# RaduAlexandru/permuto_sdf

Measured on AMD Instinct MI355X. Metric: ray-samples/sec (encode+MLP+composite), higher is better.
Workload: dtype f32 (MLP products on 2 fp16 operand pieces per fp32 value, fp32 accumulation; the 3-piece / 24-bit figure is value_fp32_equivalent_24bit)

## Files before the change

### include/psdf.h

```cpp
#ifndef PSDF_H
#define PSDF_H
#include <stdint.h>
#ifdef __cplusplus
extern "C" {
#endif

int64_t psdf_encode_convention(int which);
int psdf_encode_set_conventions(uint32_t hash_multiplier, int rank_tie_raises_later);

int psdf_encode_forward(int pos_dim, int nr_feat, int64_t N, int nr_levels, int capacity, const float* positions,
    const float* lattice, const float* scale_factor, const float* shifts, const float* window, int concat_points,
    float points_scaling, float* sliced, void* stream);

int psdf_encode_forward_mark(int pos_dim, int nr_feat, int64_t N, int nr_levels, int capacity, const float* positions,
    const float* lattice, const float* scale_factor, const float* shifts, const float* window, int concat_points,
    float points_scaling, float* sliced, unsigned char* touched_blocks, int block_rows_log2, void* stream);

int psdf_encode_backward(int pos_dim, int nr_feat, int64_t N, int nr_levels, int capacity, const float* positions,
    const float* lattice, const float* scale_factor, const float* shifts, const float* window, int concat_points,
    float points_scaling, const float* grad_sliced, float* grad_lattice, float* grad_positions, void* stream);

int64_t psdf_encode_backward_workspace_bytes(int pos_dim, int nr_feat, int64_t N, int nr_levels, int capacity);
int psdf_encode_backward_ws(int pos_dim, int nr_feat, int64_t N, int nr_levels, int capacity, const float* positions,
    const float* lattice, const float* scale_factor, const float* shifts, const float* window, int concat_points,
    float points_scaling, const float* grad_sliced, float* grad_lattice, float* grad_positions, void* workspace,
    int64_t workspace_bytes, void* stream);
int psdf_encode_backward_level_shares(int* counts, int max_levels);


int psdf_encode_double_backward(int pos_dim, int nr_feat, int64_t N, int nr_levels, int capacity, const float*
    positions, const float* lattice, const float* scale_factor, const float* shifts, const float* window, int
    concat_points, float points_scaling, const float* dd_positions, const float* grad_sliced, float* grad_lattice,
    float* grad_grad_sliced, void* stream);
int psdf_encode_double_backward_ws(int pos_dim, int nr_feat, int64_t N, int nr_levels, int capacity, const float* positions,
                                   const float* lattice, const float* scale_factor, const float* shifts, const float* window,
                                   int concat_points, float points_scaling, const float* dd_positions, const float* grad_sliced,
                                   float* grad_lattice, float* grad_grad_sliced, const float* grad_sliced_direct,
                                   void* workspace, int64_t workspace_bytes, void* stream);

int psdf_mlp_pack_f16(int n_layers, const int* dims, const float* const* weights, const float* const* biases, float* packed,
    void* stream);
int psdf_mlp_forward_f16(int n_layers, const int* dims, int64_t N, const float* X, const float* packed, float* Y, void* stream);

int psdf_neus_composite_forward(int nr_rays, const int* start_end, int equal, int fixed, int max_nr_samples, const float* sdf,
    const float* dirs, const float* gradients, const float* dt, const float* rgb, const float* inv_s, float cos_anneal_ratio,
    float* pred, float* bg, float* weights, void* stream);
int psdf_neus_composite_backward(int nr_rays, const int* start_end, int equal, int fixed, int max_nr_samples, int max_per_ray,
    const float* grad_pred, const float* grad_bg, const float* sdf, const float* dirs, const float* gradients, const float* dt,
    const float* rgb, const float* inv_s, float cos_anneal_ratio, int reference_compat, float* grad_sdf, float* grad_gradients,
    float* grad_rgb, float* grad_inv_s, void* stream);

int psdf_nerf_composite_forward(int nr_rays, const int* start_end, int equal, int fixed, int max_nr_samples, const float* raw_density,
                                const float* dt, const float* rgb, const float* fg_pred, const float* fg_bg, float* pred_bg,
                                float* pred, void* stream);
int psdf_nerf_composite_backward(int nr_rays, const int* start_end, int equal, int fixed, int max_nr_samples, int max_per_ray,
                                 const float* grad_pred, const float* fg_bg, const float* raw_density, const float* dt,
                                 const float* rgb, int reference_compat, float* grad_raw_density, float* grad_rgb,
                                 float* grad_fg_bg, void* stream);

int psdf_last_path(int family);
enum {
  PSDF_MLP_OP_FORWARD = 0,
  PSDF_MLP_OP_FORWARD_F16 = 1,
  PSDF_MLP_OP_FORWARD_WIDE_F16 = 2,
  PSDF_MLP_OP_BACKWARD = 3,
  PSDF_MLP_OP_BACKWARD_DATA = 4,
  PSDF_MLP_OP_BACKWARD_DATA_MASKED = 5,
  PSDF_MLP_OP_DOUBLE_BACKWARD = 6,
  PSDF_MLP_OP_DOUBLE_BACKWARD_PLUS = 7
};
int psdf_mlp_supported(int op, int n_layers, const int* dims);

int psdf_mlp_backward_split(int n_layers, const int* dims, int64_t N, const float* X, const float* const* weights,
    const float* const* biases, const float* dY, float* dX, float* const* dW, float* const* db, void* stream);

int psdf_mlp_backward_split_f16(int n_layers, const int* dims, int64_t N, const float* X, const float* const* weights,
    const float* const* biases, const float* dY, float* dX, float* const* dW, float* const* db, void* stream);
int psdf_mlp_backward_split_f16_form(void);
unsigned psdf_mlp_f16_range_events(void);

int psdf_mlp_forward_wide_f16(int n_layers, const int* dims, int64_t N, const float* X, const float* const* weights,
    const float* const* biases, float* Y, void* stream);
int psdf_mlp_backward_wide_form(void);
int psdf_mlp_backward_wide(int n_layers, const int* dims, int64_t N, const float* X, const float* const* weights,
    const float* const* biases, const float* dY, float* dX, float* const* dW, float* const* db, void* stream);

int psdf_lipshitz_normalize_forward(int out, int in, const float* W, const float* c, float* Wn, void* stream);
int psdf_lipshitz_normalize_backward(int out, int in, const float* W, const float* c, const float* grad_Wn, float* grad_W,
    float* grad_c, void* stream);
int psdf_lipshitz_normalize_forward_multi(int n_layers, const int* out, const int* in, const float* const* W, const float* const* c,
                                          float* const* Wn, void* stream);
int psdf_lipshitz_normalize_backward_multi(int n_layers, const int* out, const int* in, const float* const* W, const float* const* c,
                                           const float* const* grad_Wn, float* const* grad_W, float* const* grad_c, void* stream);

int psdf_neus_alpha_forward(int64_t N, const float* sdf, const float* dirs, const float* gradients, const float* dt,
    const float* inv_s, float cos_anneal_ratio, float* alpha, float* one_minus_alpha, void* stream);
int psdf_neus_alpha_backward(int64_t N, const float* grad_alpha, const float* sdf, const float* dirs, const float*
    gradients, const float* dt, const float* inv_s, float cos_anneal_ratio, float* grad_sdf, float* grad_gradients,
    float* grad_inv_s, void* stream);
int psdf_l1_loss(int64_t R, int C, const float* pred, const float* gt, const unsigned char* mask, float scale,
    float* loss, float* grad_pred, void* stream);
int psdf_eikonal_loss(int64_t N, const float* gradients, float scale, float* loss, float* grad_gradients, void* stream);
int psdf_normalize3(int64_t N, const float* x, const float* grad_y, float* out, void* stream);
int psdf_sigmoid_rows(int64_t N, int C, const float* x_fm, float* y, void* stream);
int psdf_sigmoid_rows_backward(int64_t N, int C, const float* grad_y, const float* y, float* grad_x_fm, void* stream);
int psdf_curvature_shift(int64_t N, const float* points, const float* gradients, const float* rand_directions, float
    epsilon, const float* grad_shifted, float* out, void* stream);
int psdf_curvature_loss(int64_t N, const float* gradients, const float* gradients_shifted, float scale, float* loss,
    float* grad_gradients, float* grad_gradients_shifted, void* stream);
int psdf_offsurface_loss(int64_t N, const float* sdf, float sharpness, float scale, float* loss, float* grad_sdf, void*
    stream);
int psdf_nerf_alpha_forward(int64_t N, const float* raw_density, const float* dt, float* alpha, float* one_minus_alpha,
    void* stream);
int psdf_nerf_alpha_backward(int64_t N, const float* raw_density, const float* dt, const float* grad_alpha, const float*
    grad_one_minus_alpha, float* grad_raw_density, void* stream);

int64_t psdf_mlp_packed_size(int n_layers, const int* dims);

int psdf_mlp_pack(int n_layers, const int* dims, const float* const* weights, const float* const* biases, float*
    packed, void* stream);

int psdf_mlp_forward(int n_layers, const int* dims, int64_t N, const float* X, const float* packed, float* Y, void*
    stream);

int psdf_encode_forward_masked(int pos_dim, int nr_feat, int64_t N, int nr_levels, int capacity, const float* positions,
    const float* lattice, const float* scale_factor, const float* shifts, const float* window, int concat_points, float
    points_scaling, const uint8_t* skip, float* sliced, void* stream);
int psdf_mlp_forward_masked(int n_layers, const int* dims, int64_t N, const float* X, const float* packed, const uint8_t*
    skip, float* Y, void* stream);
int psdf_mlp_backward_data_masked(int n_layers, const int* dims, int64_t N, const float* X, const float* const* weights,
    const float* const* biases, const float* dY, const uint8_t* skip, float* dX, void* stream);
int psdf_encode_backward_positions_masked(int pos_dim, int nr_feat, int64_t N, int nr_levels, int capacity, const float*
    positions, const float* lattice, const float* scale_factor, const float* shifts, const float* window, int
    concat_points, float points_scaling, const float* grad_sliced, const uint8_t* skip, float* grad_positions, void*
    stream);

int psdf_mlp_backward(int n_layers, const int* dims, int64_t N, const float* X, const float* const* weights, const
    float* const* biases, const float* dY, float* dX, float* const* dW, float* const* db, void* stream);

int psdf_mlp_double_backward(int n_layers, const int* dims, int64_t N, const float* X, const float* const* weights,
    const float* const* biases, const float* dY, const float* V, float* dX2, float* const* dW, float* const* db,
    void* stream);
int psdf_mlp_double_backward_plus(int n_layers, const int* dims, int64_t N, const float* X, const float* const* weights,
    const float* const* biases, const float* dY, const float* V, const float* dY2, float* dX2, float* const* dW,
    float* const* db, void* stream);

int psdf_encode_mlp_forward(int64_t N, int nr_levels, int capacity, const float* positions, const float* lattice,
    const float* scale_factor, const float* shifts, const float* window, int concat_points, float points_scaling,
    int n_layers, const int* dims, const float* packed, const uint8_t* skip, float* feat, float* Y, void* stream);

int psdf_adamw_step(int64_t n, float* param, const float* grad, float* exp_avg, float* exp_avg_sq, float lr, float
    beta1, float beta2, float eps, float weight_decay, int step, float grad_scale, void* stream);

int psdf_adamw_step_multi(int n_tensors, const int64_t* sizes, float* const* params, const float* const* grads, float*
    const* exp_avgs, float* const* exp_avg_sqs, float lr, float beta1, float beta2, float eps, float weight_decay, int
    step, float grad_scale, void* stream);

int psdf_adamw_step_blocks(int64_t n_blocks, int block_elems, float* param, float* grad, float* exp_avg, float*
    exp_avg_sq, unsigned char* touched, unsigned char* active, float lr, float beta1, float beta2, float eps, int step,
    float grad_scale, int zero_grad, void* stream);
int psdf_adamw_step_blocks_multi(int n_tensors, const int64_t* n_blocks, const int* block_elems, float* const* params,
    float* const* grads, float* const* exp_avgs, float* const* exp_avg_sqs, unsigned char* const* touched,
    unsigned char* const* active, const float* lr, const float* beta1, const float* beta2, const float* eps, const int* step,
    float grad_scale, int zero_grad, void* stream);


int psdf_grid_points(int count, int nr_voxels_per_dim, float extent, const float* grid_translation, const int*
    voxel_indices, uint64_t rng_state, uint64_t rng_inc, int randomize, float* out_points, void* stream);

int psdf_grid_update_with_density(int count, const int* voxel_indices, const float* density, float decay, float
    thresh, float* grid_values, uint8_t* grid_occupancy, void* stream);

int psdf_grid_update_with_sdf(int count, const int* voxel_indices, const float* sdf, int nr_voxels_per_dim, float
    extent, const float* grid_translation, float inv_s, const float* inv_s_tensor, int full_update, float thresh,
    float* grid_values, uint8_t* grid_occupancy, void* stream);

int psdf_grid_check_occupancy(int count, int nr_voxels_per_dim, float extent, const float* grid_translation, const
    uint8_t* grid_occupancy, const float* points, uint8_t* out, void* stream);

int psdf_march_form(void);
int psdf_march_samples(int use_grid, int nr_rays, int nr_voxels_per_dim, float extent, const float* grid_translation,
    const uint8_t* grid_occupancy, const float* ray_origins, const float* ray_dirs, const float* ray_t_entry, const
    float* ray_t_exit, float min_dist_between_samples, int max_nr_samples_per_ray, int max_nr_samples, uint64_t
    rng_state, uint64_t rng_inc, int jitter, float* samples_pos, float* samples_dirs, float* samples_z, float*
    samples_dt, float* ray_fixed_dt, int* ray_start_end_idx, int* cur_nr_samples, int* scratch, const uint32_t*
    coarse_mask, void* stream);

int psdf_first_hit_samples(int nr_rays, int nr_voxels_per_dim, float extent, const float* grid_translation, const
    uint8_t* grid_occupancy, const float* ray_origins, const float* ray_dirs, const float* ray_t_entry, const float*
    ray_t_exit, int max_nr_samples, float* samples_pos, float* samples_dirs, float* samples_z, float* samples_dt,
    float* ray_fixed_dt, int* ray_start_end_idx, int* cur_nr_samples, int* scratch, const uint32_t* coarse_mask,
    void* stream);

int psdf_advance_to_next_occupied_voxel(int count, int nr_voxels_per_dim, float extent, const float* grid_translation,
    const uint8_t* grid_occupancy, const float* samples_dirs, float* samples_pos, uint8_t* is_within_bounds, const
    uint32_t* coarse_mask, void* stream);

int psdf_occupancy_coarse_words(int nr_voxels_per_dim);
int psdf_occupancy_coarse_mask(int nr_voxels_per_dim, const uint8_t* grid_occupancy, uint32_t* coarse_mask, void*
    stream);

int psdf_samples_bg(int nr_rays, int nr_samples_per_ray, const float* ray_origins, const float* ray_dirs, const float*
    ray_t_exit, float sphere_radius, const float* sphere_center, uint64_t rng_state, uint64_t rng_inc, int randomize,
    int contract_3d_samples, float* samples_3d, float* samples_4d, float* samples_dirs, float* samples_z, float*
    samples_dt, float* ray_fixed_dt, int* ray_start_end_idx, void* stream);

int psdf_sphere_ray_intersection(int nr_rays, float radius, const float* center, const float* ray_origins, const
    float* ray_dirs, float* points_entry, float* t_entry, float* points_exit, float* t_exit, uint8_t* does_intersect,
    void* stream);

int psdf_sphere_rand_points_inside(int count, float radius, const float* phi, const float* costheta, const float* u,
    float* points, void* stream);

int psdf_compact_offsets(int nr_rays, const int* ray_start_end_idx, int* scratch, int* total, void* stream);

int psdf_compact_copy(int nr_rays, const int* ray_start_end_idx, const int* offsets, const float* pos, const float*
    pos4, const float* dirs, const float* z, const float* dt, const float* sdf, const float* fixed_dt, float* o_pos,
    float* o_pos4, float* o_dirs, float* o_z, float* o_dt, float* o_sdf, float* o_fixed_dt, int* o_start_end, void*
    stream);

int psdf_per_sample_ray_idx(int nr_rays, int nr_samples, const int* ray_start_end_idx, int* out, void* stream);

int psdf_spherical_harmonics(int count, int degree, const float* dirs, float* out, void* stream);

int psdf_random_rays_from_reel(int nr_rays, int nr_images, int height, int width, const float* rgb_reel, const float*
    mask_reel, const float* K_reel, const float* tf_world_cam_reel, const int* pixel_indices, const int* img_indices,
    int has_mask, float* ray_origins, float* ray_dirs, float* gt_rgb, float* gt_mask, void* stream);

int psdf_first_hit_dense(int nr_rays, int nr_voxels_per_dim, float extent, const float* grid_translation, const
    uint8_t* grid_occupancy, const float* ray_origins, const float* ray_dirs, const float* ray_t_entry, const float*
    ray_t_exit, float* pos, uint8_t* converged, const uint32_t* coarse_mask, void* stream);
int psdf_sphere_trace_step(int count, int nr_voxels_per_dim, float extent, const float* grid_translation, const
    uint8_t* grid_occupancy, const float* dirs, const float* sdf, float sdf_multiplier, float sdf_converged_thresh,
    float* pts, uint8_t* converged, const uint32_t* coarse_mask, void* stream);
int psdf_sphere_trace_step_compacted(int count, int nr_voxels_per_dim, float extent, const float* grid_translation, const
    uint8_t* grid_occupancy, const float* dirs, const float* sdf, float sdf_multiplier, float sdf_converged_thresh,
    float* pts, uint8_t* converged, uint8_t* work_flags, int* work_list, int* work_count, const uint32_t* coarse_mask,
    void* stream);

int psdf_exclusive_scan_i32(int n, const int* in, int* out, int* total, void* stream);

int psdf_cumprod_alpha2transmittance(int nr_rays, const int* start_end, int equal, int fixed, int max_nr_samples,
    const float* alpha, float* transmittance, float* bg_transmittance, void* stream);

int psdf_cumprod_alpha2transmittance_backward(int nr_rays, const int* start_end, int equal, int fixed, int
    max_nr_samples, const float* grad_bg, const float* alpha, const float* bg, const float* cumsumLV, float*
    grad_alpha, void* stream);

int psdf_integrate_with_weights(int nr_rays, const int* start_end, int equal, int fixed, int max_nr_samples, const
    float* rgb, const float* weights, float* pred, void* stream);

int psdf_integrate_with_weights_backward(int nr_rays, const int* start_end, int equal, int fixed, int max_nr_samples,
    const float* grad_pred, const float* rgb, const float* weights, float* grad_rgb, float* grad_weights, int
    reference_compat, void* stream);

int psdf_sum_over_each_ray(int nr_rays, const int* start_end, int equal, int fixed, int max_nr_samples, int channels,
    const float* values, float* sum_per_ray, float* sum_per_sample, void* stream);

int psdf_sum_over_each_ray_backward(int nr_rays, const int* start_end, int equal, int fixed, int max_nr_samples, int
    channels, const float* grad_per_ray, const float* grad_per_sample, float* grad_values, void* stream);

int psdf_cumsum_over_each_ray(int nr_rays, const int* start_end, int equal, int fixed, int max_nr_samples, const
    float* values, int inverse, int exclusive, float* out, void* stream);

int psdf_sdf2alpha(int nr_rays, const int* start_end, int equal, int fixed, int max_nr_samples, const float*
    ray_fixed_dt, const float* samples_dt, const float* sdf, float inv_s, int dynamic_inv_s, float inv_s_multiplier,
    float* alpha, void* stream);
int psdf_sdf_importance_cdf(int nr_rays, const int* start_end, int equal, int fixed, int max_nr_samples, const float* ray_fixed_dt,
                            const float* samples_dt, const float* sdf, float inv_s, int dynamic_inv_s, float inv_s_multiplier,
                            float* cdf, void* stream);

int psdf_compute_dt(int nr_rays, const int* start_end, int equal, int fixed, int max_nr_samples, const float*
    samples_z, const float* ray_t_exit, int use_ray_t_exit, float* dt, void* stream);

int psdf_volume_render_nerf(int nr_rays, const int* start_end, int equal, int fixed, int max_nr_samples, const float*
    rgb, const float* density, const float* samples_z, const float* samples_dt, float* pred_rgb, float* pred_depth,
    float* bg_transmittance, float* weight_per_sample, void* stream);

int psdf_volume_render_nerf_backward(int nr_rays, const int* start_end, int equal, int fixed, int max_nr_samples,
    const float* grad_pred_rgb, const float* grad_bg_transmittance, const float* pred_rgb, const float*
    bg_transmittance, const float* rgb, const float* density, const float* samples_dt, float* grad_rgb, float*
    grad_density, void* stream);

int psdf_importance_sample(int nr_rays, const int* start_end, int equal, int fixed, int max_nr_samples, const float*
    ray_origins, const float* ray_dirs, const float* ray_fixed_dt, const float* samples_z, const float* cdf, int
    nr_importance_samples, uint64_t rng_state, uint64_t rng_inc, int jitter, float* out_pos, float* out_dirs, float*
    out_z, void* stream);

int psdf_combine_uniform_samples_with_imp(int nr_rays, const int* uni_start_end, int uni_equal, int uni_fixed, int
    uni_max_nr_samples, const float* ray_origins, const float* ray_dirs, const float* ray_t_exit, const float*
    uni_fixed_dt, const float* uni_z, const float* uni_sdf, int has_sdf, int nr_imp, const float* imp_z, const float*
    imp_sdf, int out_max_nr_samples, float* out_pos, float* out_dirs, float* out_z, float* out_dt, float* out_sdf,
    float* out_fixed_dt, int* out_start_end, int* out_cur_nr_samples, int* scratch, void* stream);

int psdf_mesh_classify(const float* vol, const uint8_t* valid, float level, int X, int Y, int Z, int xbase, int nplanes, int p0,
    int p1, int c0, int c1, uint8_t* mask, int32_t* vcount, int32_t* tcount, void* stream);
int psdf_mesh_emit_vertices(const float* vol, float level, int X, int Y, int Z, int xbase, int nplanes, int p0, int p1, const
    uint8_t* mask, const int32_t* vincl, int64_t v_off, float* verts, int64_t* edges, float* normals, void* stream);
int psdf_mesh_emit_faces(const float* vol, const uint8_t* valid, float level, int X, int Y, int Z, int xbase, int nplanes, int c0,
    int c1, const uint8_t* mask, const int32_t* vincl, const int32_t* tincl, int32_t* faces, void* stream);
int psdf_mesh_grid_points(int nx, int Y, int Z, int x0, int64_t first, int64_t count, const float* xs, const float* ys, const
    float* zs, float* points, void* stream);
int psdf_mesh_sparse_mask(int64_t count, int nr_voxels_per_dim, float extent, const float* grid_translation, const uint8_t*
    grid_occupancy, const float* points, float h, uint8_t* valid, uint8_t* skip, void* stream);

int psdf_mesh_eval_tile_capacity(void);
int psdf_mesh_eval_grid_plan(const double* lo, const double* hi, int64_t n_points, double min_edge, int64_t cell_budget, float*
    origin_edge, int* dims, int64_t* cells, int64_t* query_blocks);
int psdf_mesh_sample_count(const float* V, int64_t nV, const int32_t* F, int64_t nF, double density, int32_t* counts, int32_t*
    overflow, void* stream);
int psdf_mesh_sample_emit(const float* V, int64_t nV, const int32_t* F, int64_t nF, double density, const int64_t* incl, float*
    samples, void* stream);
int psdf_mesh_eval_cell_keys(const float* points, int64_t n, const float* origin_edge, const int* dims, int block_log2, int32_t*
    keys, void* stream);
int psdf_mesh_eval_cell_ranges(const int32_t* sorted_keys, int64_t n, int64_t cells, int32_t* start, void* stream);
int psdf_mesh_thin_sweep(const float* points, const int32_t* rank, const int32_t* keys, int64_t n, const int32_t* cell_start,
    const float* origin_edge, const int* dims, float radius, uint8_t* state, int32_t* undecided, void* stream);
int psdf_mesh_nn_cooperative(const float* queries, int64_t nq, const int32_t* query_block_start, const float* refs, int64_t nr,
    const int32_t* cell_start, const float* origin_edge, const int* dims, float max_dist, float* dist, int32_t* idx, uint8_t*
    open, int32_t* nr_open, void* stream);
int psdf_mesh_nn_ring(const float* queries, int64_t nq, const float* refs, int64_t nr, const int32_t* cell_start, const float*
    origin_edge, const int* dims, float max_dist, float* dist, int32_t* idx, const uint8_t* open, void* stream);

#ifdef __cplusplus
}
#endif
#endif
```

### permuto_sdf_amd/csrc/mlp.hip

```cpp
#include "psdf_common.h"

#include "mlp_device.h"
#include "mlp_dispatch.h"

namespace {

struct PackArgs {
  MlpPlan plan;
  const float* W[MAXL];
  const float* b[MAXL];
};

__global__ void mlp_pack_kernel(PackArgs a, float* __restrict__ packed) {
  const int e = blockIdx.x * blockDim.x + threadIdx.x;
  const MlpPlan& p = a.plan;
  if (e >= p.total) return;
  int l = 0;
#pragma unroll
  for (int i = 1; i < MAXL; i++)
    if (i < p.n_layers && e >= p.w_off[i]) l = i;
  const int out_d = p.dims[l + 1], in_d = p.dims[l];
  const bool last = (l == p.n_layers - 1);
  float v = 0.f;
  if (e >= p.b_off[l]) {
    const int row = e - p.b_off[l];
    if (row < out_d) v = a.b[l][row];
  } else {
    const int q = e - p.w_off[l];
    int row, col;
    if (l == 0) {
      const int lane = q % WS, s = (q / WS) % p.in_steps0, to = (q / WS) / p.in_steps0;
      row = (lane < 64) ? 32 * to + (lane & 31) : (1 << 20);
      col = 2 * s + (lane >> 5);
    } else if (last && p.final_dot) {
      const int h = q & 1, r = (q >> 1) & 15, ti = (q >> 5) % p.tiles[l], o = (q >> 5) / p.tiles[l];
      row = o;
      col = 32 * ti + row_of(r, h);
    } else {
      const int j = q & 3, lane = (q >> 2) & 63, rq = (q >> 8) & 3, pr = q >> 10;
      const int r = 4 * rq + j, ti = pr % p.tiles[l], to = pr / p.tiles[l];
      row = 32 * to + (lane & 31);
      col = 32 * ti + row_of(r, lane >> 5);
    }
    if (row < out_d && col < in_d) v = a.W[l][(int64_t)row * in_d + col];
  }
  packed[e] = v;
}

__global__ void mlp_pack_split_kernel(PackArgs a, SplitPlan sp, float* __restrict__ packed, int f16) {
  const int w = blockIdx.x * blockDim.x + threadIdx.x;
  const MlpPlan& p = a.plan;
  if (w >= sp.total_rec * 4) return;
  uint32_t* dst = reinterpret_cast<uint32_t*>(packed + sp.base);
  const int nl = p.n_layers;
  const int rec = w >> 2;
  if (rec >= sp.tail_rec) {
    const int f = w - sp.tail_rec * 4;
    float v = 0.f;
    for (int l = 0; l < nl; l++) {
      const bool dot = (l == nl - 1) && p.final_dot;
      const int nb = dot ? 4 : p.tiles[l + 1] * 32;
      if (f >= sp.b_off[l] && f < sp.b_off[l] + nb) {
        const int row = f - sp.b_off[l];
        if (row < p.dims[l + 1]) v = a.b[l][row];
      }
      if (dot && f >= sp.wf_off && f < sp.wf_off + p.dims[nl] * p.tiles[l] * 32) {
        const int q = f - sp.wf_off;
        const int h = q & 1, r = (q >> 1) & 15, ti = (q >> 5) % p.tiles[l], o = (q >> 5) / p.tiles[l];
        const int col = 32 * ti + row_of(r, h);
        if (col < p.dims[l]) v = a.W[l][(int64_t)o * p.dims[l] + col];
      }
    }
    dst[w] = __float_as_uint(v);
    return;
  }
  int l = 0;
  for (int i = 1; i < nl; i++) {
    const bool dot = (i == nl - 1) && p.final_dot;
    if (!dot && rec >= sp.w_rec[i]) l = i;
  }
  const int local = rec - sp.w_rec[l];
  const int lane = local & 63, piece = (local >> 6) % 3, s = (local / 192) % sp.ns[l], to = (local / 192) / sp.ns[l];
  const int row = 32 * to + (lane & 31), hh = lane >> 5;
  uint32_t out = 0;
  for (int e = 0; e < 2; e++) {
    const int j = 2 * (w & 3) + e;
    const int col = l == 0 ? 16 * s + 8 * hh + j : 32 * (s >> 1) + row_of(8 * (s & 1) + j, hh);
    float v = 0.f;
    if (row < p.dims[l + 1] && col < p.dims[l]) v = a.W[l][(int64_t)row * p.dims[l] + col];
    uint32_t pc[3];
    if (f16) split2h_bits(v, pc);
    else split3(v, pc);
    out |= pc[piece] << (16 * e);
  }
  dst[w] = out;
}

template <int T1, int T2, int T3>
struct Net {
  static constexpr int NH = (T3 > 0) ? 3 : 2;
  static constexpr int TL = (T3 > 0) ? T3 : T2;
};

template <int T1, int T2, int T3, int OUT_T, bool FINAL_DOT>
__global__ void __launch_bounds__(PSDF_BLOCK, 2)
    mlp_fwd_kernel(MlpPlan p, int64_t N, const float* __restrict__ X, const float* __restrict__ packed,
                   const unsigned char* __restrict__ skip, float* __restrict__ Y) {
  extern __shared__ __align__(16) float lds[];
  for (int i = threadIdx.x; i < p.total; i += PSDF_BLOCK) lds[i] = packed[i];
  __syncthreads();
  const int lane = threadIdx.x & 63, wave = __builtin_amdgcn_readfirstlane((int)(threadIdx.x >> 6));
  const int h = lane >> 5, sl = lane & 31;
  const int K0 = p.dims[0];
  const int OUT = p.dims[p.n_layers];
  const int64_t ntiles = (N + 31) / 32;
  for (int64_t tile = (int64_t)blockIdx.x * 4 + wave; tile < ntiles; tile += (int64_t)gridDim.x * 4) {
    asm volatile("" ::: "memory");
    const int64_t n = tile * 32 + sl;
    const int64_t nc = n < N ? n : N - 1;
    if (skip && __ballot(n < N && !skip[nc]) == 0) continue;
    f32x16 h1[T1];
    init_bias<T1>(h1, lds + p.b_off[0], h);
    {
      const float* __restrict__ w0 = lds + p.w_off[0];
      const int steps = p.in_steps0;
      constexpr int XC = 16;
      for (int s0 = 0; s0 < steps; s0 += XC) {
        float xb[XC];
#pragma unroll
        for (int i = 0; i < XC; i++) {
          const int k = 2 * (s0 + i) + h;
          xb[i] = (s0 + i < steps && k < K0) ? X[(int64_t)k * N + nc] : 0.f;
        }
#pragma unroll
        for (int i = 0; i < XC; i++) {
          if (s0 + i < steps) {
#pragma unroll
            for (int to = 0; to < T1; to++)
              h1[to] = __builtin_amdgcn_mfma_f32_32x32x2f32(w0[(to * steps + s0 + i) * WS + lane], xb[i], h1[to], 0, 0, 0);
          }
        }
      }
    }
    apply_gelu<T1>(h1);
    f32x16 h2[T2];
    init_bias<T2>(h2, lds + p.b_off[1], h);
    dense_chain<T1, T2>(h1, h2, lds + p.w_off[1], lane);
    apply_gelu<T2>(h2);
    constexpr int TL = (T3 > 0) ? T3 : T2;
    f32x16 hl[TL];
    if constexpr (T3 > 0) {
      init_bias<T3>(hl, lds + p.b_off[2], h);
      dense_chain<T2, T3>(h2, hl, lds + p.w_off[2], lane);
      apply_gelu<T3>(hl);
    } else {
#pragma unroll
      for (int t = 0; t < T2; t++) hl[t] = h2[t];
    }
    const int lf = p.n_layers - 1;
    if constexpr (FINAL_DOT) {
      const float* __restrict__ wf = lds + p.w_off[lf];
      for (int o = 0; o < OUT; o++) {
        float acc = 0.f;
#pragma unroll
        for (int ti = 0; ti < TL; ti++)
#pragma unroll
          for (int r = 0; r < 16; r++) acc = fmaf(wf[((o * TL + ti) * 16 + r) * 2 + h], hl[ti][r], acc);
        acc += __shfl_xor(acc, 32, 64);
        acc += lds[p.b_off[lf] + o];
        if (h == 0 && n < N) Y[(int64_t)o * N + n] = acc;
      }
    } else {
      f32x16 y[OUT_T];
      init_bias<OUT_T>(y, lds + p.b_off[lf], h);
      dense_chain<TL, OUT_T>(hl, y, lds + p.w_off[lf], lane);
      if (n < N) {
#pragma unroll
        for (int to = 0; to < OUT_T; to++)
#pragma unroll
          for (int r = 0; r < 16; r++) {
            const int row = 32 * to + row_of(r, h);
            if (row < OUT) Y[(int64_t)row * N + n] = y[to][r];
          }
      }
    }
  }
}

#define GELU_SPLIT(T_, H_)                        \
  do {                                            \
    if constexpr (F16) apply_gelu_packed<T_>(H_); \
    else apply_gelu_scalar<T_>(H_);               \
  } while (0)
template <int T1, int T2, int T3, int OUT_T, bool FINAL_DOT, int CH, bool F16 = false>
__global__ void __launch_bounds__(PSDF_BLOCK, 2)
    mlp_fwd_split_kernel(MlpPlan p, SplitPlan sp, int64_t N, const float* __restrict__ X,
                         const float* __restrict__ packed, const unsigned char* __restrict__ skip,
                         float* __restrict__ Y) {
  extern __shared__ __align__(16) u32x4 simg[];
  {
    const u32x4* __restrict__ src = reinterpret_cast<const u32x4*>(packed + sp.base);
    for (int i = threadIdx.x; i < sp.total_rec; i += PSDF_BLOCK) simg[i] = src[i];
  }
  __syncthreads();
  const float* tail = reinterpret_cast<const float*>(simg + sp.tail_rec);
  const int lane = threadIdx.x & 63, wave = __builtin_amdgcn_readfirstlane((int)(threadIdx.x >> 6));
  const int h = lane >> 5, sl = lane & 31;
  const int K0 = p.dims[0];
  const int OUT = p.dims[p.n_layers];
  const int ns0 = sp.ns[0];
  const int64_t ntiles = (N + 31) / 32;
  for (int64_t tile = (int64_t)blockIdx.x * 4 + wave; tile < ntiles; tile += (int64_t)gridDim.x * 4) {
    asm volatile("" ::: "memory");
    const int64_t n = tile * 32 + sl;
    const int64_t nc = n < N ? n : N - 1;
    if (skip && __ballot(n < N && !skip[nc]) == 0) continue;
    f32x16 h1[T1];
    init_bias4<T1>(h1, tail + sp.b_off[0], h);
    const float* __restrict__ xl = X + nc + (h ? (int64_t)8 * N : (int64_t)0);
    for (int s0 = 0; s0 < ns0; s0 += CH) {
      float xs[CH][8];
#pragma unroll
      for (int i = 0; i < CH; i++) {
        const int sb = 16 * (s0 + i);
        if (sb + 16 <= K0) {
#pragma unroll
          for (int j = 0; j < 8; j++) xs[i][j] = xl[(int64_t)(sb + j) * N];
        } else if (sb < K0) {
#pragma unroll
          for (int j = 0; j < 8; j++) {
            const int k = sb + 8 * h + j;
            const float v = X[(int64_t)(k < K0 ? k : K0 - 1) * N + nc];
            xs[i][j] = k < K0 ? v : 0.f;
          }
        } else {
#pragma unroll
          for (int j = 0; j < 8; j++) xs[i][j] = 0.f;
        }
      }
#pragma unroll
      for (int i = 0; i < CH; i++) {
        const int s = s0 + i < ns0 ? s0 + i : ns0 - 1;
        split_mac<T1, F16>(h1, xs[i], simg + sp.w_rec[0] + s * 192, ns0, lane);
      }
    }
    GELU_SPLIT(T1, h1);
    f32x16 h2[T2];
    init_bias4<T2>(h2, tail + sp.b_off[1], h);
    split_chain<T1, T2, F16>(h1, h2, simg + sp.w_rec[1], lane);
    GELU_SPLIT(T2, h2);
    constexpr int TL = (T3 > 0) ? T3 : T2;
    f32x16 hl[TL];
    if constexpr (T3 > 0) {
      init_bias4<T3>(hl, tail + sp.b_off[2], h);
      split_chain<T2, T3, F16>(h2, hl, simg + sp.w_rec[2], lane);
      GELU_SPLIT(T3, hl);
    } else {
#pragma unroll
      for (int t = 0; t < T2; t++) hl[t] = h2[t];
    }
    const int lf = p.n_layers - 1;
    if constexpr (FINAL_DOT) {
      const float* __restrict__ wf = tail + sp.wf_off;
      for (int o = 0; o < OUT; o++) {
        float acc = 0.f;
#pragma unroll
        for (int ti = 0; ti < TL; ti++)
#pragma unroll
          for (int r = 0; r < 16; r++) acc = fmaf(wf[((o * TL + ti) * 16 + r) * 2 + h], hl[ti][r], acc);
        acc += __shfl_xor(acc, 32, 64);
        acc += tail[sp.b_off[lf] + o];
        if (h == 0 && n < N) Y[(int64_t)o * N + n] = acc;
      }
    } else {
      f32x16 y[OUT_T];
      init_bias4<OUT_T>(y, tail + sp.b_off[lf], h);
      split_chain<TL, OUT_T, F16>(hl, y, simg + sp.w_rec[lf], lane);
      if (n < N) {
#pragma unroll
        for (int to = 0; to < OUT_T; to++)
#pragma unroll
          for (int r = 0; r < 16; r++) {
            const int row = 32 * to + row_of(r, h);
            if (row < OUT) Y[(int64_t)row * N + n] = y[to][r];
          }
      }
    }
  }
}

template <int T1, int T2, int T3, int OUT_T, bool FINAL_DOT, int CH, bool F16 = false>
int launch_fwd_split_ch(const MlpPlan& p, const SplitPlan& sp, int64_t N, const float* X, const float* packed,
                     const unsigned char* skip, float* Y, hipStream_t st) {
  const size_t shmem = (size_t)sp.total_rec * 16;
  auto kern = mlp_fwd_split_kernel<T1, T2, T3, OUT_T, FINAL_DOT, CH, F16>;
  if (shmem > 64 * 1024) {
    hipError_t e = hipFuncSetAttribute((const void*)kern, hipFuncAttributeMaxDynamicSharedMemorySize, (int)shmem);
    if (e != hipSuccess) return (int)e;
  }
  const int64_t ntiles = (N + 31) / 32;
  int64_t blocks = (ntiles + 3) / 4;
  const int64_t cap = 256 * 4;
  if (blocks > cap) blocks = cap;
  hipLaunchKernelGGL(kern, dim3((unsigned)blocks), dim3(PSDF_BLOCK), shmem, st, p, sp, N, X, packed, skip, Y);
  PSDF_LAUNCH_CHECK();
  return PSDF_OK;
}

template <int T1, int T2, int T3, int OUT_T, bool FINAL_DOT>
int launch_fwd_split(const MlpPlan& p, const SplitPlan& sp, int64_t N, const float* X, const float* packed,
                     const unsigned char* skip, float* Y, hipStream_t st, bool f16 = false) {
  if constexpr (T1 == 2 && T2 == 2 && T3 == 2 && OUT_T == 1 && FINAL_DOT) {
    if (f16) {
      switch (sp.ns[0]) {
        case 1: return launch_fwd_split_ch<T1, T2, T3, OUT_T, FINAL_DOT, 1, true>(p, sp, N, X, packed, skip, Y, st);
        case 2: return launch_fwd_split_ch<T1, T2, T3, OUT_T, FINAL_DOT, 2, true>(p, sp, N, X, packed, skip, Y, st);
        case 3: return launch_fwd_split_ch<T1, T2, T3, OUT_T, FINAL_DOT, 3, true>(p, sp, N, X, packed, skip, Y, st);
        default: return launch_fwd_split_ch<T1, T2, T3, OUT_T, FINAL_DOT, 4, true>(p, sp, N, X, packed, skip, Y, st);
      }
    }
  } else if (f16) {
    return PSDF_ERR_UNSUPPORTED;
  }
  switch (sp.ns[0]) {
    case 1: return launch_fwd_split_ch<T1, T2, T3, OUT_T, FINAL_DOT, 1>(p, sp, N, X, packed, skip, Y, st);
    case 2: return launch_fwd_split_ch<T1, T2, T3, OUT_T, FINAL_DOT, 2>(p, sp, N, X, packed, skip, Y, st);
    case 3: return launch_fwd_split_ch<T1, T2, T3, OUT_T, FINAL_DOT, 3>(p, sp, N, X, packed, skip, Y, st);
    default: return launch_fwd_split_ch<T1, T2, T3, OUT_T, FINAL_DOT, 4>(p, sp, N, X, packed, skip, Y, st);
  }
}

template <int T1, int T2, int T3, int OUT_T, bool FINAL_DOT>
int launch_fwd(const MlpPlan& p, int64_t N, const float* X, const float* packed, const unsigned char* skip, float* Y,
               hipStream_t st) {
  const size_t shmem = (size_t)p.total * sizeof(float);
  auto kern = mlp_fwd_kernel<T1, T2, T3, OUT_T, FINAL_DOT>;
  if (!fwd_fits(p)) return PSDF_ERR_UNSUPPORTED;
  if (shmem > 64 * 1024) {
    hipError_t e = hipFuncSetAttribute((const void*)kern, hipFuncAttributeMaxDynamicSharedMemorySize, (int)shmem);
    if (e != hipSuccess) return (int)e;
  }
  const int64_t ntiles = (N + 31) / 32;
  int64_t blocks = (ntiles + 3) / 4;
  const int64_t cap = 256 * 4;
  if (blocks > cap) blocks = cap;
  hipLaunchKernelGGL(kern, dim3((unsigned)blocks), dim3(PSDF_BLOCK), shmem, st, p, N, X, packed, skip, Y);
  PSDF_LAUNCH_CHECK();
  return PSDF_OK;
}


}

extern "C" {

int64_t psdf_mlp_packed_size(int n_layers, const int* dims) {
  MlpPlan p;
  if (make_plan(n_layers, dims, p) != PSDF_OK) return PSDF_ERR_ARG;
  SplitPlan sp;
  make_split_plan(p, sp);
  return sp.ok ? (int64_t)sp.base + (int64_t)sp.total_rec * 4 : (int64_t)p.total;
}

static int mlp_pack_impl(int n_layers, const int* dims, const float* const* weights, const float* const* biases,
                         float* packed, void* stream, int f16) {
  PackArgs a;
  int rc = make_plan(n_layers, dims, a.plan);
  if (rc != PSDF_OK) return rc;
  if (f16 && !baseline_split_shape(n_layers, dims, 64, 4)) return PSDF_ERR_UNSUPPORTED;
  for (int l = 0; l < MAXL; l++) {
    a.W[l] = l < n_layers ? weights[l] : nullptr;
    a.b[l] = l < n_layers ? biases[l] : nullptr;
  }
  hipLaunchKernelGGL(mlp_pack_kernel, dim3(psdf_blocks(a.plan.total, 256)), dim3(256), 0, (hipStream_t)stream, a,
                     packed);
  PSDF_LAUNCH_CHECK();
  SplitPlan sp;
  make_split_plan(a.plan, sp);
  if (sp.ok) {
    hipLaunchKernelGGL(mlp_pack_split_kernel, dim3(psdf_blocks(sp.total_rec * 4, 256)), dim3(256), 0,
                       (hipStream_t)stream, a, sp, packed, f16);
    PSDF_LAUNCH_CHECK();
  } else if (f16) {
    return PSDF_ERR_UNSUPPORTED;
  }
  return PSDF_OK;
}

int psdf_mlp_pack(int n_layers, const int* dims, const float* const* weights, const float* const* biases,
                  float* packed, void* stream) {
  return mlp_pack_impl(n_layers, dims, weights, biases, packed, stream, 0);
}

int psdf_mlp_pack_f16(int n_layers, const int* dims, const float* const* weights, const float* const* biases,
                      float* packed, void* stream) {
  return mlp_pack_impl(n_layers, dims, weights, biases, packed, stream, 1);
}

static int mlp_forward_impl(int n_layers, const int* dims, int64_t N, const float* X, const float* packed,
                            const unsigned char* skip, float* Y, void* stream, bool f16 = false) {
  MlpPlan p;
  int rc = make_plan(n_layers, dims, p);
  if (rc != PSDF_OK) return rc;
  if (N == 0) return PSDF_OK;
  if (N < 0 || !X || !packed || !Y) return PSDF_ERR_ARG;
  hipStream_t st = (hipStream_t)stream;
  const int t1 = p.tiles[1], t2 = p.tiles[2], t3 = (n_layers == 4) ? p.tiles[3] : 0, to = p.tiles[n_layers];
  if (n_layers != 3 && n_layers != 4) return PSDF_ERR_UNSUPPORTED;
  if (f16 && !baseline_split_shape(n_layers, dims, 64, 4)) return PSDF_ERR_UNSUPPORTED;
  SplitPlan sp;
  make_split_plan(p, sp);
#define CASE(A, B, C, O, D, FWD, S, F16)                                        \
  PSDF_IF(FWD, if (t1 == A && t2 == B && t3 == C && to == O && p.final_dot == D) { \
    if (f16 && !F16) return PSDF_ERR_UNSUPPORTED;                               \
    if constexpr (S) {                                                          \
      if (sp.ok) {                                                              \
        psdf::g_last_path[psdf::PATH_MLP_FWD] = f16 ? 3 : 2;                    \
        return launch_fwd_split<A, B, C, O, D>(p, sp, N, X, packed, skip, Y, st, f16); \
      }                                                                         \
    }                                                                           \
    if (f16) return PSDF_ERR_UNSUPPORTED;                                       \
    psdf::g_last_path[psdf::PATH_MLP_FWD] = 1;                                  \
    return launch_fwd<A, B, C, O, D>(p, N, X, packed, skip, Y, st);             \
  })
  PSDF_MLP32_ROWS(CASE)
#undef CASE
  return PSDF_ERR_UNSUPPORTED;
}


int psdf_mlp_forward(int n_layers, const int* dims, int64_t N, const float* X, const float* packed, float* Y,
                     void* stream) {
  return mlp_forward_impl(n_layers, dims, N, X, packed, nullptr, Y, stream);
}

int psdf_mlp_forward_f16(int n_layers, const int* dims, int64_t N, const float* X, const float* packed, float* Y,
                         void* stream) {
  return mlp_forward_impl(n_layers, dims, N, X, packed, nullptr, Y, stream, true);
}

int psdf_mlp_forward_masked(int n_layers, const int* dims, int64_t N, const float* X, const float* packed,
                            const unsigned char* skip, float* Y, void* stream) {
  return mlp_forward_impl(n_layers, dims, N, X, packed, skip, Y, stream);
}

}
```

### permuto_sdf_amd/mlp.py

```python
import ctypes
import math

import torch

from . import _lib as L


def _dims_array(dims):
    return (ctypes.c_int * len(dims))(*dims)


def packed_size(dims):
    n = L.lib().psdf_mlp_packed_size
    n.restype = ctypes.c_int64
    r = n(L.c_i(len(dims) - 1), _dims_array(dims))
    if r < 0:
        raise L.PsdfError("psdf_mlp_packed_size: bad layer widths %s" % (dims,))
    return int(r)


(OP_FORWARD, OP_FORWARD_F16, OP_FORWARD_WIDE_F16, OP_BACKWARD, OP_BACKWARD_DATA, OP_BACKWARD_DATA_MASKED, OP_DOUBLE_BACKWARD,
 OP_DOUBLE_BACKWARD_PLUS) = range(8)
_SUPPORTED = {}


def supported(op, dims):
    key = (op, tuple(dims))
    r = _SUPPORTED.get(key)
    if r is None:
        r = _SUPPORTED[key] = L.lib().psdf_mlp_supported(L.c_i(op), L.c_i(len(dims) - 1), _dims_array(dims)) == 1
    return r


def f16_forward_supported(dims):
    return supported(OP_FORWARD_F16, dims)


def pack_params(dims, weights, biases, f16=False):
    n_layers = len(dims) - 1
    L.require_cuda(*weights)
    packed = torch.empty(packed_size(dims), dtype=torch.float32, device=weights[0].device)
    ws = [w.detach().contiguous() for w in weights]
    bs = [b.detach().contiguous() for b in biases]
    W = (ctypes.c_void_p * n_layers)(*[w.data_ptr() for w in ws])
    B = (ctypes.c_void_p * n_layers)(*[b.data_ptr() for b in bs])
    L.call("psdf_mlp_pack_f16" if f16 else "psdf_mlp_pack", L.c_i(n_layers), _dims_array(dims), W, B, L.ptr(packed), L.stream())
    return packed


def mlp_forward_raw(dims, x_fm, packed, skip=None, out=None, f16=False):
    N = x_fm.shape[1]
    y = out if out is not None else torch.empty((dims[-1], N), dtype=torch.float32, device=x_fm.device)
    if f16:
        assert skip is None
        L.call("psdf_mlp_forward_f16", L.c_i(len(dims) - 1), _dims_array(dims), L.c_l(N), L.ptr(x_fm), L.ptr(packed), L.ptr(y),
               L.stream())
    elif skip is None:
        L.call("psdf_mlp_forward", L.c_i(len(dims) - 1), _dims_array(dims), L.c_l(N), L.ptr(x_fm), L.ptr(packed), L.ptr(y),
               L.stream())
    else:
        L.call("psdf_mlp_forward_masked", L.c_i(len(dims) - 1), _dims_array(dims), L.c_l(N), L.ptr(x_fm), L.ptr(packed),
               L.ptr(skip), L.ptr(y), L.stream())
    return y


_wide_f16_fn = None


def mlp_forward_wide_f16_raw(dims, x_fm, weights, biases, out=None):
    global _wide_f16_fn
    if len(dims) != 5:
        return None
    if _wide_f16_fn is None:
        _wide_f16_fn = L.lib().psdf_mlp_forward_wide_f16
        _wide_f16_fn.restype = ctypes.c_int
    N = x_fm.shape[1]
    y = out if out is not None else torch.empty((dims[-1], N), dtype=torch.float32, device=x_fm.device)
    arr = lambda ts: (ctypes.c_void_p * 4)(*[t.data_ptr() for t in ts])
    ws = [w.detach() if w.is_contiguous() else w.detach().contiguous() for w in weights]
    bs = [b.detach() for b in biases]
    rc = _wide_f16_fn(L.c_i(4), _dims_array(dims), L.c_l(N), L.ptr(x_fm), arr(ws), arr(bs), L.ptr(y), L.stream())
    if rc == -2:
        return None
    if rc != 0:
        L.check(rc, "psdf_mlp_forward_wide_f16")
    return y


def _grad_views(dims, flat=None, dev=None):
    n_layers = len(dims) - 1
    sizes = [dims[l + 1] * dims[l] for l in range(n_layers)] + [dims[l + 1] for l in range(n_layers)]
    offs, tot = [], 0
    for sz in sizes:
        offs.append(tot)
        tot += (sz + 3) & ~3
    if flat is None:
        flat = torch.zeros(tot, dtype=torch.float32, device=dev)
    dWs = [flat[offs[l]:offs[l] + sizes[l]].view(dims[l + 1], dims[l]) for l in range(n_layers)]
    dbs = [flat[offs[n_layers + l]:offs[n_layers + l] + sizes[n_layers + l]] for l in range(n_layers)]
    return flat, dWs, dbs


def _zero_grads(dims, dev):
    _, dWs, dbs = _grad_views(dims, dev=dev)
    return dWs, dbs


class GradBuffer:

    def __init__(self, dims, device):
        self.flat, self.dWs, self.dbs = _grad_views(dims, dev=device)
        self.accumulating = False

    def accumulate(self):
        from .encoding import _Flag
        return _Flag(self, "accumulating")

    def zero(self):
        self.flat.zero_()


def mlp_backward_raw(dims, x_fm, weights, biases, gy_fm, need_dx=True, need_dw=True, into=None):
    assert gy_fm is not None or not need_dw
    N = x_fm.shape[1]
    n_layers = len(dims) - 1
    dev = x_fm.device
    ws = [w.detach().contiguous() for w in weights]
    bs = [b.detach().contiguous() for b in biases]
    dx = torch.empty((dims[0], N), dtype=torch.float32, device=dev) if need_dx else None
    Wp = (ctypes.c_void_p * n_layers)(*[w.data_ptr() for w in ws])
    Bp = (ctypes.c_void_p * n_layers)(*[b.data_ptr() for b in bs])
    if need_dw:
        dWs, dbs = into if into is not None else _zero_grads(dims, dev)
        W = (ctypes.c_void_p * n_layers)(*[w.data_ptr() for w in dWs])
        B = (ctypes.c_void_p * n_layers)(*[b.data_ptr() for b in dbs])
    else:
        dWs, dbs, W, B = [], [], None, None
    L.call("psdf_mlp_backward", L.c_i(n_layers), _dims_array(dims), L.c_l(N), L.ptr(x_fm), Wp, Bp, L.ptr(gy_fm),
           L.ptr(dx), W, B, L.stream())
    return dx, dWs, dbs


def backward_supported(dims):
    return supported(OP_BACKWARD, dims)


_ANNOUNCED = set()


def torch_fallback_allowed(module=None):
    import os
    return bool(getattr(module, "allow_torch_fallback", False)) or os.environ.get("PSDF_MLP_TORCH_FALLBACK") == "1"


def _announce(kind, dims, module=None):
    if not torch_fallback_allowed(module):
        raise L.PsdfError("permuto_sdf_amd: no fused %s kernel is instantiated for the MLP widths %s (csrc/mlp_dispatch.h lists "
                          "the instantiated widths).  Refusing to fall back to torch/rocBLAS silently: pass allow_torch_fallback=True "
                          "to FusedMLP or set PSDF_MLP_TORCH_FALLBACK=1 to opt in." % (kind, list(dims)))
    key = (kind, tuple(dims))
    if key not in _ANNOUNCED:
        _ANNOUNCED.add(key)
        import warnings
        warnings.warn("permuto_sdf_amd: no fused %s kernel is instantiated for the MLP widths %s; using torch autograd over "
                      "rocBLAS on the GPU for it (csrc/mlp_dispatch.h lists the instantiated widths)" % (kind, list(dims)),
                      RuntimeWarning, stacklevel=3)


def _torch_gpu_backward(dims, x_fm, weights, biases, gy_fm, need_dx, module=None):
    _announce("backward", dims, module)
    n_layers = len(dims) - 1
    with torch.enable_grad():
        x = x_fm.t().detach().requires_grad_(need_dx)
        ws = [w.detach().requires_grad_(True) for w in weights]
        bs = [b.detach().requires_grad_(True) for b in biases]
        h = x
        for i in range(n_layers):
            h = torch.nn.functional.linear(h, ws[i], bs[i])
            if i < n_layers - 1:
                h = torch.nn.functional.gelu(h)
        outs = torch.autograd.grad(h, ([x] if need_dx else []) + ws + bs, gy_fm.t())
    k = 1 if need_dx else 0
    dx = outs[0].t().contiguous() if need_dx else None
    return dx, list(outs[k:k + n_layers]), list(outs[k + n_layers:])


def _torch_gpu_double_backward(dims, x_fm, weights, biases, gy_fm, v_fm, module=None):
    _announce("double backward", dims, module)
    n_layers = len(dims) - 1
    with torch.enable_grad():
        x = x_fm.t().detach().requires_grad_(True)
        ws = [w.detach().requires_grad_(True) for w in weights]
        bs = [b.detach().requires_grad_(True) for b in biases]
        h = x
        for i in range(n_layers):
            h = torch.nn.functional.linear(h, ws[i], bs[i])
            if i < n_layers - 1:
                h = torch.nn.functional.gelu(h)
        (gx,) = torch.autograd.grad(h, x, gy_fm.t(), create_graph=True)
        outs = torch.autograd.grad(gx, [x] + ws + bs, v_fm.t(), allow_unused=True)
    outs = [o if o is not None else torch.zeros_like(t) for o, t in zip(outs, [x] + ws + bs)]
    return outs[0].t().contiguous(), list(outs[1:1 + n_layers]), list(outs[1 + n_layers:])


class _InputGradOnly:

    def __init__(self, modules):
        self.modules = modules

    def __enter__(self):
        self.prev = [m._input_grad_only for m in self.modules]
        for m in self.modules:
            m._input_grad_only = True

    def __exit__(self, *exc):
        for m, v in zip(self.modules, self.prev):
            m._input_grad_only = v


def input_gradient_only(*modules):
    if not modules:
        raise TypeError("input_gradient_only(net, ...): name the FusedMLP modules whose parameter gradients are to be skipped")
    return _InputGradOnly(modules)


def _grad_buffer_open(module):
    gb = getattr(module, "grad_buffer", None)
    return gb if (gb is not None and gb.accumulating and not torch.is_grad_enabled()) else None


class _FusedMLPFunc(torch.autograd.Function):

    @staticmethod
    def forward(ctx, module, x, *params):
        n_layers = module.n_layers
        weights, biases = params[:n_layers], params[n_layers:]
        x_fm = x.t()
        if not x_fm.is_contiguous():
            x_fm = x_fm.contiguous()
        y = None
        if supported(OP_FORWARD_WIDE_F16, module.dims):
            y = mlp_forward_wide_f16_raw(module.dims, x_fm, weights, biases)
        if y is None:
            packed = pack_params(module.dims, weights, biases)
            y = mlp_forward_raw(module.dims, x_fm, packed)
        ctx.module = module
        ctx.n_layers = n_layers
        ctx.save_for_backward(x, *weights, *biases)
        return y.t()

    @staticmethod
    def backward(ctx, gy):
        x = ctx.saved_tensors[0]
        params = ctx.saved_tensors[1:]
        if getattr(ctx.module, "_input_grad_only", False):
            outs = _FusedMLPBackFunc.apply(ctx.module, (ctx.needs_input_grad[1], False), x, gy, *params)
            return (None, outs[0] if ctx.needs_input_grad[1] else None, *([None] * len(params)))
        gb = _grad_buffer_open(ctx.module)
        if gb is not None:
            outs = _FusedMLPBackFunc.apply(ctx.module, (ctx.needs_input_grad[1], True, True), x, gy, *params)
            return (None, outs[0] if ctx.needs_input_grad[1] else None, *([None] * len(params)))
        outs = _FusedMLPBackFunc.apply(ctx.module, ctx.needs_input_grad[1], x, gy, *params)
        dx = outs[0] if ctx.needs_input_grad[1] else None
        return (None, dx, *outs[1:])


class _FusedMLPBackFunc(torch.autograd.Function):

    @staticmethod
    def forward(ctx, module, need_dx, x, gy, *params):
        need_dw, buffered = True, False
        if isinstance(need_dx, tuple):
            need_dx, need_dw, buffered = (tuple(need_dx) + (False,))[:3]
        n_layers = module.n_layers
        weights, biases = params[:n_layers], params[n_layers:]
        x_fm = x.t()
        if not x_fm.is_contiguous():
            x_fm = x_fm.contiguous()
        gy_fm = gy.t()
        if not gy_fm.is_contiguous():
            gy_fm = gy_fm.contiguous()
        if not need_dw and supported(OP_BACKWARD_DATA, module.dims):
            dx, dWs, dbs = mlp_backward_raw(module.dims, x_fm, weights, biases, gy_fm, need_dx=need_dx, need_dw=False)
        elif backward_supported(module.dims):
            gb = module.grad_buffer if buffered else None
            dx, dWs, dbs = mlp_backward_raw(module.dims, x_fm, weights, biases, gy_fm, need_dx=need_dx,
                                            into=(gb.dWs, gb.dbs) if gb is not None else None)
            if not need_dw or buffered:
                dWs, dbs = [], []
        else:
            dx, dWs, dbs = _torch_gpu_backward(module.dims, x_fm, weights, biases, gy_fm, need_dx, module)
            if buffered:
                gb = module.grad_buffer
                for dst, src in zip(gb.dWs + gb.dbs, list(dWs) + list(dbs)):
                    dst.add_(src)
                dWs, dbs = [], []
        ctx.module, ctx.n_layers = module, n_layers
        ctx.set_materialize_grads(False)
        ctx.save_for_backward(x_fm, gy_fm, *weights, *biases)
        if dx is None:
            dx_out = L.zero_scalar(x.device)
            ctx.mark_non_differentiable(dx_out)
        else:
            dx_out = dx.t()
        return (dx_out, *dWs, *dbs)

    @staticmethod
    def backward(ctx, g_dx, *g_params):
        n_layers = ctx.n_layers
        x_fm, gy_fm = ctx.saved_tensors[0], ctx.saved_tensors[1]
        weights = ctx.saved_tensors[2:2 + n_layers]
        biases = ctx.saved_tensors[2 + n_layers:]
        if any(g is not None for g in g_params):
            raise NotImplementedError("FusedMLP: differentiating through the parameter gradients (dW, db) is not implemented")
        if ctx.needs_input_grad[3] and g_dx is not None:
            raise NotImplementedError("FusedMLP: the upstream gradient of the MLP output requires grad (a differentiable "
                                      "function of the output is being differentiated twice); the J_x v term is not implemented")
        if g_dx is None:
            return (None,) * (4 + 2 * n_layers)
        v_fm = g_dx.t()
        if not v_fm.is_contiguous():
            v_fm = v_fm.contiguous()
        gb = _grad_buffer_open(ctx.module)
        if gb is not None:
            dX, _, _ = mlp_double_backward(ctx.module.dims, x_fm, weights, biases, gy_fm, v_fm, into=(gb.dWs, gb.dbs),
                                           module=ctx.module)
            return (None, None, dX.t(), None, *([None] * (2 * n_layers)))
        dX, dWs, dbs = mlp_double_backward(ctx.module.dims, x_fm, weights, biases, gy_fm, v_fm, module=ctx.module)
        return (None, None, dX.t(), None, *dWs, *dbs)


def double_backward_supported(dims):
    return supported(OP_DOUBLE_BACKWARD, dims)


def double_backward_plus_supported(dims):
    return supported(OP_DOUBLE_BACKWARD_PLUS, dims)


def mlp_double_backward(dims, x_fm, weights, biases, gy_fm, v_fm, into=None, module=None, gy2_fm=None):
    if gy2_fm is not None:
        assert double_backward_plus_supported(dims), dims
    if gy_fm is None and not double_backward_supported(dims):
        gy_fm = torch.zeros((dims[-1], x_fm.shape[1]), dtype=torch.float32, device=x_fm.device)
        gy_fm[0].fill_(1.0)
    if not double_backward_supported(dims):
        dX, dWs, dbs = _torch_gpu_double_backward(dims, x_fm, weights, biases, gy_fm, v_fm, module)
        if into is not None:
            for dst, src in zip(list(into[0]) + list(into[1]), list(dWs) + list(dbs)):
                if src is not None:
                    dst.add_(src)
            dWs, dbs = into
        return dX, dWs, dbs
    N = x_fm.shape[1]
    n_layers = len(dims) - 1
    dev = x_fm.device
    ws = [w.detach().contiguous() for w in weights]
    bs = [b.detach().contiguous() for b in biases]
    dx2 = torch.empty((dims[0], N), dtype=torch.float32, device=dev)
    dWs, dbs = into if into is not None else _zero_grads(dims, dev)
    Wp = (ctypes.c_void_p * n_layers)(*[w.data_ptr() for w in ws])
    Bp = (ctypes.c_void_p * n_layers)(*[b.data_ptr() for b in bs])
    W = (ctypes.c_void_p * n_layers)(*[w.data_ptr() for w in dWs])
    B = (ctypes.c_void_p * n_layers)(*[b.data_ptr() for b in dbs])
    if gy2_fm is not None:
        L.call("psdf_mlp_double_backward_plus", L.c_i(n_layers), _dims_array(dims), L.c_l(N), L.ptr(x_fm), Wp, Bp, L.ptr(gy_fm),
# ... 169 lines not shown
```

Measured before the change: 976.5 million.

## Add 8-wave workgroup form for split MLP forward and occupancy-based grid cap

Turns the split-MLP forward kernel body into a template over waves per workgroup and adds an 8-wave variant (launch bounds W*64, 4). That variant is used for the 2/2/2-tile final-dot configuration when there are enough tiles per CU. Larger workgroups spread the shared-memory weight image copy across more waves, so each copy feeds more tiles. The grid cap now comes from the occupancy API and the device CU count instead of a hardcoded 1024 blocks. The trade-off is more register pressure under the stricter launch bounds, and fewer resident workgroups if shared memory limits occupancy.

```diff
diff --git a/include/psdf.h b/include/psdf.h
--- a/include/psdf.h
+++ b/include/psdf.h
@@ -41,6 +41,9 @@
 int psdf_mlp_pack_f16(int n_layers, const int* dims, const float* const* weights, const float* const* biases, float* packed,
     void* stream);
 int psdf_mlp_forward_f16(int n_layers, const int* dims, int64_t N, const float* X, const float* packed, float* Y, void* stream);
+
+int psdf_mlp_forward_set_form(int waves);
+int psdf_mlp_forward_last_form(void);
 
 int psdf_neus_composite_forward(int nr_rays, const int* start_end, int equal, int fixed, int max_nr_samples, const float* sdf,
     const float* dirs, const float* gradients, const float* dt, const float* rgb, const float* inv_s, float cos_anneal_ratio,
diff --git a/permuto_sdf_amd/csrc/mlp.hip b/permuto_sdf_amd/csrc/mlp.hip
--- a/permuto_sdf_amd/csrc/mlp.hip
+++ b/permuto_sdf_amd/csrc/mlp.hip
@@ -192,15 +192,14 @@
     if constexpr (F16) apply_gelu_packed<T_>(H_); \
     else apply_gelu_scalar<T_>(H_);               \
   } while (0)
-template <int T1, int T2, int T3, int OUT_T, bool FINAL_DOT, int CH, bool F16 = false>
-__global__ void __launch_bounds__(PSDF_BLOCK, 2)
-    mlp_fwd_split_kernel(MlpPlan p, SplitPlan sp, int64_t N, const float* __restrict__ X,
-                         const float* __restrict__ packed, const unsigned char* __restrict__ skip,
-                         float* __restrict__ Y) {
+template <int T1, int T2, int T3, int OUT_T, bool FINAL_DOT, int CH, bool F16, int W>
+__device__ __forceinline__ void mlp_fwd_split_body(const MlpPlan& p, const SplitPlan& sp, int64_t N, const float* __restrict__ X,
+                                                   const float* __restrict__ packed, const unsigned char* __restrict__ skip,
+                                                   float* __restrict__ Y) {
   extern __shared__ __align__(16) u32x4 simg[];
   {
     const u32x4* __restrict__ src = reinterpret_cast<const u32x4*>(packed + sp.base);
-    for (int i = threadIdx.x; i < sp.total_rec; i += PSDF_BLOCK) simg[i] = src[i];
+    for (int i = threadIdx.x; i < sp.total_rec; i += W * 64) simg[i] = src[i];
   }
   __syncthreads();
   const float* tail = reinterpret_cast<const float*>(simg + sp.tail_rec);
@@ -210,7 +209,7 @@
   const int OUT = p.dims[p.n_layers];
   const int ns0 = sp.ns[0];
   const int64_t ntiles = (N + 31) / 32;
-  for (int64_t tile = (int64_t)blockIdx.x * 4 + wave; tile < ntiles; tile += (int64_t)gridDim.x * 4) {
+  for (int64_t tile = (int64_t)blockIdx.x * W + wave; tile < ntiles; tile += (int64_t)gridDim.x * W) {
     asm volatile("" ::: "memory");
     const int64_t n = tile * 32 + sl;
     const int64_t nc = n < N ? n : N - 1;
@@ -290,21 +289,98 @@
 }
 
 template <int T1, int T2, int T3, int OUT_T, bool FINAL_DOT, int CH, bool F16 = false>
-int launch_fwd_split_ch(const MlpPlan& p, const SplitPlan& sp, int64_t N, const float* X, const float* packed,
-                     const unsigned char* skip, float* Y, hipStream_t st) {
+__global__ void __launch_bounds__(PSDF_BLOCK, 2)
+    mlp_fwd_split_kernel(MlpPlan p, SplitPlan sp, int64_t N, const float* __restrict__ X,
+                         const float* __restrict__ packed, const unsigned char* __restrict__ skip,
+                         float* __restrict__ Y) {
+  mlp_fwd_split_body<T1, T2, T3, OUT_T, FINAL_DOT, CH, F16, 4>(p, sp, N, X, packed, skip, Y);
+}
+
+template <int T1, int T2, int T3, int OUT_T, bool FINAL_DOT, int CH, bool F16, int W>
+__global__ void __launch_bounds__(W * 64, 4)
+    mlp_fwd_split_wg_kernel(MlpPlan p, SplitPlan sp, int64_t N, const float* __restrict__ X,
+                            const float* __restrict__ packed, const unsigned char* __restrict__ skip,
+                            float* __restrict__ Y) {
+  mlp_fwd_split_body<T1, T2, T3, OUT_T, FINAL_DOT, CH, F16, W>(p, sp, N, X, packed, skip, Y);
+}
+
+constexpr int SPLIT_WIDE_W = 8;
+constexpr int SPLIT_WIDE_MIN_TILES_PER_CU = 16;
+
+template <int T1, int T2, int T3, int OUT_T, bool FINAL_DOT, int W>
+constexpr bool split_wide_built = T1 == 2 && T2 == 2 && (T3 == 2 || T3 == 0) && OUT_T == 1 && FINAL_DOT && W == SPLIT_WIDE_W;
+
+int g_fwd_form_forced = 0;
+int g_fwd_form_last = 0;
+
+int mlp_device_cus() {
+  static int cus[64] = {};
+  int dev = 0;
+  if (hipGetDevice(&dev) != hipSuccess || dev < 0 || dev >= 64) return 256;
+  if (cus[dev] == 0) {
+    int n = 0;
+    if (hipDeviceGetAttribute(&n, hipDeviceAttributeMultiprocessorCount, dev) != hipSuccess || n <= 0) n = 256;
+    cus[dev] = n;
+  }
+  return cus[dev];
+}
+
+template <int W, auto KERN>
+int launch_fwd_split_form(const MlpPlan& p, const SplitPlan& sp, int64_t N, const float* X, const float* packed,
+                          const unsigned char* skip, float* Y, hipStream_t st) {
+  const auto kern = KERN;
   const size_t shmem = (size_t)sp.total_rec * 16;
-  auto kern = mlp_fwd_split_kernel<T1, T2, T3, OUT_T, FINAL_DOT, CH, F16>;
   if (shmem > 64 * 1024) {
     hipError_t e = hipFuncSetAttribute((const void*)kern, hipFuncAttributeMaxDynamicSharedMemorySize, (int)shmem);
     if (e != hipSuccess) return (int)e;
   }
+  struct Round { size_t shmem; int per_cu; };
+  static Round rounds[64] = {};
+  int dev = 0;
+  if (hipGetDevice(&dev) != hipSuccess || dev < 0 || dev >= 64) dev = 0;
+  Round& r = rounds[dev];
+  if (r.shmem != shmem || r.per_cu <= 0) {
+    int per_cu = 0;
+    if (hipOccupancyMaxActiveBlocksPerMultiprocessor(&per_cu, kern, W * 64, shmem) != hipSuccess || per_cu <= 0) {
+      (void)hipGetLastError();
+      per_cu = 2;
+    }
+    r = Round{shmem, per_cu};
+  }
+  const int round_per_cu = r.per_cu;
   const int64_t ntiles = (N + 31) / 32;
-  int64_t blocks = (ntiles + 3) / 4;
-  const int64_t cap = 256 * 4;
+  int64_t blocks = (ntiles + W - 1) / W;
+  const int64_t cap = (int64_t)round_per_cu * mlp_device_cus();
   if (blocks > cap) blocks = cap;
-  hipLaunchKernelGGL(kern, dim3((unsigned)blocks), dim3(PSDF_BLOCK), shmem, st, p, sp, N, X, packed, skip, Y);
+  hipLaunchKernelGGL(kern, dim3((unsigned)blocks), dim3(W * 64), shmem, st, p, sp, N, X, packed, skip, Y);
   PSDF_LAUNCH_CHECK();
+  g_fwd_form_last = W;
   return PSDF_OK;
+}
+
+template <int T1, int T2, int T3, int OUT_T, bool FINAL_DOT, int CH, bool F16, int W>
+int launch_fwd_split_wide(const MlpPlan& p, const SplitPlan& sp, int64_t N, const float* X, const float* packed,
+                          const unsigned char* skip, float* Y, hipStream_t st) {
+  if constexpr (split_wide_built<T1, T2, T3, OUT_T, FINAL_DOT, W>)
+    return launch_fwd_split_form<W, mlp_fwd_split_wg_kernel<T1, T2, T3, OUT_T, FINAL_DOT, CH, F16, W>>(p, sp, N, X, packed, skip, Y,
+                                                                                                         st);
+  else
+    return PSDF_ERR_UNSUPPORTED;
+}
+
+template <int T1, int T2, int T3, int OUT_T, bool FINAL_DOT, int CH, bool F16 = false>
+int launch_fwd_split_ch(const MlpPlan& p, const SplitPlan& sp, int64_t N, const float* X, const float* packed,
+                     const unsigned char* skip, float* Y, hipStream_t st) {
+  constexpr bool WIDE = split_wide_built<T1, T2, T3, OUT_T, FINAL_DOT, SPLIT_WIDE_W>;
+  int form = g_fwd_form_forced;
+  if (form == 0) {
+    const int64_t ntiles = (N + 31) / 32;
+    form = WIDE && ntiles >= (int64_t)SPLIT_WIDE_MIN_TILES_PER_CU * mlp_device_cus() ? SPLIT_WIDE_W : 4;
+  }
+  if (form == 4)
+    return launch_fwd_split_form<4, mlp_fwd_split_kernel<T1, T2, T3, OUT_T, FINAL_DOT, CH, F16>>(p, sp, N, X, packed, skip, Y, st);
+  if (form == 8) return launch_fwd_split_wide<T1, T2, T3, OUT_T, FINAL_DOT, CH, F16, 8>(p, sp, N, X, packed, skip, Y, st);
+  return launch_fwd_split_wide<T1, T2, T3, OUT_T, FINAL_DOT, CH, F16, 16>(p, sp, N, X, packed, skip, Y, st);
 }
 
 template <int T1, int T2, int T3, int OUT_T, bool FINAL_DOT>
@@ -444,4 +520,12 @@
   return mlp_forward_impl(n_layers, dims, N, X, packed, skip, Y, stream);
 }
 
-}
+int psdf_mlp_forward_set_form(int waves) {
+  if (waves != 0 && waves != 4 && waves != 8 && waves != 16) return PSDF_ERR_ARG;
+  g_fwd_form_forced = waves;
+  return PSDF_OK;
+}
+
+int psdf_mlp_forward_last_form(void) { return g_fwd_form_last; }
+
+}
diff --git a/permuto_sdf_amd/mlp.py b/permuto_sdf_amd/mlp.py
--- a/permuto_sdf_amd/mlp.py
+++ b/permuto_sdf_amd/mlp.py
@@ -62,6 +62,14 @@
         L.call("psdf_mlp_forward_masked", L.c_i(len(dims) - 1), _dims_array(dims), L.c_l(N), L.ptr(x_fm), L.ptr(packed),
                L.ptr(skip), L.ptr(y), L.stream())
     return y
+
+
+def set_forward_form(waves):
+    L.call("psdf_mlp_forward_set_form", L.c_i(waves))
+
+
+def last_forward_form():
+    return int(L.lib().psdf_mlp_forward_last_form())
 
 
 _wide_f16_fn = None
```

Result: faster. 989.5 million (median of 6 runs) (+1.3%).
